# nipponjo/tts-arabic-pytorch

Hardware: AMD Instinct MI355X
Metric: audio samples/sec (FastPitch+HiFi-GAN, synthetic 64-phoneme inputs) (higher is better)
Workload: dtype f32

## Files before the change

include/ttsamd.h:

```cpp
#ifndef TTSAMD_H
#define TTSAMD_H

#include <stdint.h>

#ifdef __cplusplus
extern "C" {
#endif

#define TTSAMD_OK 0
#define TTSAMD_EINVAL (-1)
#define TTSAMD_EHIP (-2)
#define TTSAMD_ENOMEM (-3)

typedef struct ttsamd_tensor {
    const char* name;
    const float* data;
    int32_t ndim;
    int64_t shape[4];
} ttsamd_tensor;

typedef struct ttsamd_hifigan_cfg {
    int32_t num_mels;
    int32_t upsample_initial_channel;
    int32_t n_ups;
// ... 273 lines not shown
int32_t ttsamd_conv_last_launch(int32_t* route, int32_t* ksplit);
int32_t ttsamd_conv1d_route(int32_t batch, int32_t cin, int32_t cout, int32_t k, int32_t dilation, int32_t lin, float in_slope,
                            int32_t relu_out, int32_t has_res, int32_t mode, int64_t splitk_floats, int32_t* route, int32_t* ksplit);
int64_t ttsamd_convt_packed_floats(int32_t cin, int32_t cout, int32_t u);
int64_t ttsamd_convt_wino_packed_floats(int32_t cin, int32_t cout, int32_t u);
int32_t ttsamd_convt_wino_pack_weight(const float* w, const float* bias, int32_t cin, int32_t cout, int32_t u, float* out);
int32_t ttsamd_conv_transpose1d(const float* x, const float* w, const float* bias, const int64_t* lens, int32_t batch, int32_t cin,
                                int32_t cout, int32_t u, int32_t lin, float in_slope, float* y, float* packed, void* stream);

int64_t ttsamd_resblock_pair_packed_floats(int32_t channels, int32_t k, int32_t variant);
int32_t ttsamd_resblock_pair(const float* x, float* y, const float* w1, const float* b1, const float* w2, const float* b2,
                             int32_t channels, int32_t k, int32_t dil, const int64_t* lens, int32_t len_mul, int32_t L,
                             int32_t batch, int32_t mode, float div, float slope, int32_t variant, float* packed, int64_t packed_floats,
                             void* stream);

int64_t ttsamd_resblock2_packed_floats(int32_t channels, int32_t k, int32_t variant);
int32_t ttsamd_resblock2(const float* x, float* y, const float* w1, const float* b1, const float* w2, const float* b2, int32_t channels,
                         int32_t k, int32_t dil1, int32_t dil2, const int64_t* lens, int32_t len_mul, int32_t L, int32_t batch, int32_t mode,
                         float div, float slope, int32_t variant, float* packed, int64_t packed_floats, void* stream);

int32_t ttsamd_bfo_pack(const float* x, int32_t batch, int32_t channels, int32_t len, float slope, void* out, void* stream);
int32_t ttsamd_bfo_unpack(const void* in, int32_t batch, int32_t channels, int32_t len, float slope, float* out, void* stream);
int64_t ttsamd_bfo_weight_elems(int32_t cout, int32_t cin, int32_t k, int32_t up);
int32_t ttsamd_bfo_pack_weight(const float* w, int32_t cout, int32_t cin, int32_t k, int32_t up, uint16_t* out);
int32_t ttsamd_bfo_conv1d(const void* x, const void* w_packed, const float* bias, const void* res, const void* sum_in,
                          const int64_t* lens, int32_t len_mul, int32_t batch, int32_t cin, int32_t cout, int32_t k,
                          int32_t dilation, int32_t up, int32_t len_in, int32_t mode, float div, float res_slope,
                          float out_slope, void* y, float* y_f32, const float* res_f32, void* stream);
int32_t ttsamd_bfo_resblock_pair(const void* x, const void* w1, const float* b1, const void* w2, const float* b2,
                                 const void* sum_in, const int64_t* lens, int32_t len_mul, int32_t batch, int32_t channels,
// ... 125 lines not shown
```

tts-arabic-pytorch_amd/csrc/api.hip:

```cpp
#include <cerrno>
#include <cstdio>
#include <cstdlib>
#include <cstring>
#include <algorithm>
#include <atomic>
#include <mutex>
#include <string>
#include <vector>

#include "kernels.hpp"

namespace ttsamd {

static thread_local std::string g_err;

void set_error(const char* fmt, ...) {
    char buf[1024];
    va_list ap;
    va_start(ap, fmt);
    vsnprintf(buf, sizeof(buf), fmt, ap);
    va_end(ap);
    g_err = buf;
}

// ... 1009 lines not shown
                               channels, k, channels, packed + 2 * n + i * nw44);
            TTS_CHECK_HIP(hipGetLastError());
        }
        rc = launch_fused_pair4(channels, x, y, packed + 2 * n, b1, packed + 2 * n + nw44, b2, k, dil, lens, len_mul, L, batch, mode, div,
                                slope, s, 7);
    } else if (variant == -1) {
        rc = 0;
    } else {
        set_error("resblock_pair: variant %d (1: first generation, 2 / 3: second generation with 256- / 128-column blocks, 4 / 5: 256 columns + Winograd phase B / both phases, 6: C = 32 with both phases on Winograd F(4,3), 7: ... on its seven-point groups, k = 7 / 11)", variant);
        rc = TTSAMD_EINVAL;
    }
    prof_end(s);
    return rc;
}

int64_t ttsamd_resblock2_packed_floats(int32_t channels, int32_t k, int32_t variant) {
    if (channels < 1 || k < 1 || (variant != 1 && variant != 2)) return 0;
    return 2 * (int64_t)channels * k * channels;
}

int32_t ttsamd_resblock2(const float* x, float* y, const float* w1, const float* b1, const float* w2, const float* b2, int32_t channels,
                         int32_t k, int32_t dil1, int32_t dil2, const int64_t* lens, int32_t len_mul, int32_t L, int32_t batch, int32_t mode,
                         float div, float slope, int32_t variant, float* packed, int64_t packed_floats, void* stream) {
    TTS_REQUIRE(x && y && w1 && b1 && w2 && b2 && packed && channels % 32 == 0 && channels >= 32 && k >= 1 && batch >= 1 && L >= 1 &&
                len_mul >= 1 && mode >= 0 && mode <= 2 && x != y, "resblock2: bad argument");
    TTS_REQUIRE(variant == 1 || variant == 2, "resblock2: variant %d (1: two single-conv launches, 2: both convs in one launch)", variant);
    TTS_REQUIRE(packed_floats >= ttsamd_resblock2_packed_floats(channels, k, variant),
                "resblock2: `packed` holds %lld floats, C = %d, k = %d needs %lld (ttsamd_resblock2_packed_floats)", (long long)packed_floats,
                channels, k, (long long)ttsamd_resblock2_packed_floats(channels, k, variant));
    if (variant == 1) {
// ... 82 lines not shown
```

tts-arabic-pytorch_amd/csrc/common.hpp:

```cpp
#pragma once
#include <hip/hip_runtime.h>
#include <stdint.h>
#include <atomic>
#include <cstdarg>
#include <cstdio>
#include <cstdlib>
#include <string>

#include "../../include/ttsamd.h"

namespace ttsamd {

void set_error(const char* fmt, ...);

#define TTS_CHECK_HIP(expr)                                                         \
    do {                                                                            \
        hipError_t e_ = (expr);                                                     \
        if (e_ != hipSuccess) {                                                     \
            ttsamd::set_error("%s failed: %s (%s:%d)", #expr, hipGetErrorString(e_), \
                              __FILE__, __LINE__);                                  \
            return TTSAMD_EHIP;                                                     \
        }                                                                           \
    } while (0)

// ... 21 lines not shown
    e = hipFuncSetAttribute(fn, hipFuncAttributeMaxDynamicSharedMemorySize, bytes);
    if (e == hipSuccess && dev >= 0 && dev < 64) done.fetch_or(1ull << dev, std::memory_order_release);
    return e;
}

#define TTS_OPTIONS(X)                                                                                     \
    X(HIFIGAN_STREAMS, 0, 0, 1)    \
    X(WINO, 0, 0, 1)                                              \
    X(WINO2, 0, 0, 31)             \
    X(WINO4, 0, 0, 255)            \
    X(FUSED_PAIR, 0, 0, 1)                   \
    X(FUSED2, 0, 0, 1)                                           \
    X(FUSED2_MASK, 1, 0, 0x1ff)               \
    X(FUSED2_MASK_N1, 1, 0, 0x1ff)          \
    X(FUSED2_WB, 0, 0, 2)                     \
    X(PAIR4, 0, 0, 2)              \
    X(CONVT, 0, 0, 1)                              \
    X(CONVT_WINO, 0, 0, 2)         \
    X(BFO, 0, 0, 1)                \
    X(BFO_CHAIN, 0, 0, 1)                           \
    X(BFO_CHAIN7, 0, 0, 1)                                 \
    X(BFO_FF, 0, 0, 1)                              \
    X(BFO_SPLITK, 0, 0, 1)                                              \
    X(BFO_SMALL_TILES, 0, 0, 1)            \
    X(BF16_ATTN, 0, 0, 1)                                         \
    X(BF16_PACKED_T, 0, 0, 1)                   \
    X(ATT_RA, 0, 1, 4)                             \
    X(ATT_SPLIT, 0, 0, 1)                      \
    X(XCD_W, 0, 0, 1)                            \
    X(XCD_WMAX_KB, 0, 0, 1 << 20)     \
    X(DEEP_SPLITK, 0, 0, 1)        \
// ... 98 lines not shown
                         int u, int kt, int L, int len_mul, float in_slope, bool convt_ok, hipStream_t stream, const float* w_wino = nullptr,
                         const float* bias_wino = nullptr);
bool convt_wino_packable(int cin, int cout, int u);
void pack_convt_wino_weight(const float* w, const float* bias, int cin, int cout, int u, float* out_w, float* out_bias);
bool convt_wino_supported(const ConvParams& p, const float* w_wino, const float* bias_wino);
int32_t launch_convt_wino(const ConvParams& p, const float* w_wino, const float* bias_wino, hipStream_t stream);
bool fused_pair_supported(int32_t channels, int32_t k, int32_t dil, int32_t L, const float* x, const float* y);
int32_t launch_fused_pair(int32_t channels, const float* x, float* y, const float* w1, const float* b1, const float* w2,
                          const float* b2, int32_t k, int32_t dil, const int64_t* lens, int32_t len_mul, int32_t L, int32_t batch,
                          int32_t mode, float div, float slope, hipStream_t stream);
bool fused_pair2_supported(int32_t channels, int32_t k, int32_t dil, int32_t L, const float* x, const float* y, int32_t ntw);
int32_t launch_fused_pair2(int32_t channels, const float* x, float* y, const float* w1, const float* b1, const float* w2,
                           const float* b2, int32_t k, int32_t dil, const int64_t* lens, int32_t len_mul, int32_t L, int32_t batch,
                           int32_t mode, float div, float slope, int32_t ntw, hipStream_t stream, const float* w2_wino = nullptr,
                           const float* w1_wino = nullptr);
bool fused_pair4_supported(int32_t channels, int32_t k, int32_t dil, int32_t L, const float* x, const float* y);
int32_t launch_fused_pair4(int32_t channels, const float* x, float* y, const float* w1_wino4, const float* b1, const float* w2_wino4,
                           const float* b2, int32_t k, int32_t dil, const int64_t* lens, int32_t len_mul, int32_t L, int32_t batch,
                           int32_t mode, float div, float slope, hipStream_t stream, int32_t points = 6);
bool resblock2_conv_supported(int32_t channels, int32_t k, int32_t dil, int32_t L, const float* x, const float* y);
int32_t launch_resblock2_conv(int32_t channels, const float* x, float* y, const float* w, const float* b, int32_t k, int32_t dil,
                              const int64_t* lens, int32_t len_mul, int32_t L, int32_t batch, int32_t mode, float div, float slope,
                              hipStream_t stream);
bool resblock2_pair_supported(int32_t channels, int32_t k, int32_t d1, int32_t d2, int32_t L, const float* x, const float* y);
int32_t launch_resblock2_pair(int32_t channels, const float* x, float* y, const float* w1, const float* b1, const float* w2,
                              const float* b2, int32_t k, int32_t d1, int32_t d2, const int64_t* lens, int32_t len_mul, int32_t L,
                              int32_t batch, int32_t mode, float div, float slope, hipStream_t stream);
int32_t launch_wino(const ConvParams& p, hipStream_t stream);
void pack_wino_weight(const float* w, int cout, int cin, float* out);
int wino2_groups(int k);
// ... 64 lines not shown
```

tts-arabic-pytorch_amd/csrc/hifigan.hip:

```cpp
#include <cmath>
#include <cstring>
#include <cstdlib>
#include <map>
#include <mutex>
#include <string>
#include <vector>

#include "kernels.hpp"
#include "bfo.hpp"

namespace ttsamd {

constexpr unsigned kFused2Mask = 0x00F;
constexpr int kPair4MinK = 7;
constexpr unsigned kPair44Mask = 0x3;
constexpr unsigned kFused2MaskN1 = 0x000;
constexpr int64_t kFused2SmallColumns = 2 * 256 * 252;

constexpr unsigned kResblock2PairMask = 0x00;

static bool resblock2_pair_choice(unsigned mask, int32_t channels, int32_t k, int32_t d1, int32_t d2, int32_t L, const float* x,
                                  const float* y) {
    const int ci = channels == 32 ? 0 : (channels == 64 ? 1 : -1);
    const int ki = k == 3 ? 0 : (k == 5 ? 1 : (k == 7 ? 2 : -1));
    if (ci < 0 || ki < 0 || !(mask & (1u << (3 * ci + ki)))) return false;
    return resblock2_pair_supported(channels, k, d1, d2, L, x, y);
}

struct ConvW {
    int64_t w_off = 0, b_off = 0;
// ... 392 lines not shown
    struct Join {
        bool on; hipStream_t a, b;
        ~Join() { if (on) { (void)hipStreamSynchronize(a); (void)hipStreamSynchronize(b); } }
    } join{false, bs[1], bs[2]};
    const auto fail = [&](int32_t rc) { join.on = multi && rc != 0; return rc; };

    ConvParams p;
    std::memset(&p, 0, sizeof(p));
    p.batch = B;
    p.lens_in = lens; p.lens_out = lens;
    p.n_phase = 1; p.div = 1.f;
    p.splitk_ws = splitks[0]; p.splitk_floats = kSplitKFloats;
    const bool pack_t = default_precision() == 1 && opt_int(OPT_BF16_PACKED_T, 1) != 0;
    const Fused2Switches f2sw = read_fused2_switches();
    const bool fused_ok = default_precision() == 0 && opt_int(OPT_FUSED_PAIR, 1) != 0;
    const bool convt_ok = opt_int(OPT_CONVT, 1) != 0;
    const unsigned rb2_mask = (unsigned)opt_int(OPT_RESBLOCK2_PAIR, kResblock2PairMask);
    bool in_section = false;
    int pack_io = 0;
    auto conv = [&](const ConvW& cw, const float* x, hipStream_t st, float* y, const float* res, int L, int mul,
                    int dil, float slope, int mode, float div) -> int32_t {
        p.x = x; p.x_bs = (int64_t)cw.cin * L; p.x_cs = L;
        p.w = h->dev + cw.w_off; p.bias = h->dev + cw.b_off;
        p.w_bf16 = h->dev16 + cw.w16_off; p.precision = default_precision();
        p.w_wino = cw.ww_off >= 0 ? h->dev + cw.ww_off : nullptr;
        p.w_wino4 = (cw.ww4_off >= 0 && cw.cout >= 64) ? h->dev + cw.ww4_off : nullptr;
        p.w_wino44 = (cw.ww44_off >= 0 && cw.cout >= 64) ? h->dev + cw.ww44_off : nullptr;
        p.y = y; p.y_bs = (int64_t)cw.cout * L; p.y_cs = L; p.y_ts = 1;
        p.res = res; p.r_bs = (int64_t)cw.cout * L; p.r_cs = L;
        p.len_in_mul = mul; p.len_out_mul = mul; p.Lin = L; p.Nout = L;
// ... 172 lines not shown
                if (multi && j > 0) HG_CHECK_HIP(hipStreamWaitEvent(st, h->ev_done[j - 1], 0));
                if (in_section) prof_add(fl); else prof_begin(st, fl);
                rc2 = launch_resblock2_conv(w2.cin, Tb, cur, h->dev + w2.w_off, h->dev + w2.b_off, w2.k, d2, lens, mul, L, B, mode, div,
                                            0.1f, st);
                if (!in_section) prof_end(st);
                HG_TRY(rc2);
            }
            if (multi) HG_CHECK_HIP(hipEventRecord(h->ev_done[j], st));
        }
        for (int j = 0; !h->rb2 && j < cfg.n_kernels; ++j) {
            hipStream_t st = bs[j % 3];
            float *Tb = Tbs[j % 3], *R = Rs[j % 3];
            p.splitk_ws = splitks[j % 3];
            if (multi && j > 0) HG_CHECK_HIP(hipStreamWaitEvent(st, h->ev_fork, 0));
            const float* src = ups_out;
            for (int m = 0; m < cfg.n_dilations; ++m) {
                const int li = (i * cfg.n_kernels + j) * cfg.n_dilations + m;
                const int d = cfg.resblock_dilations[j][m];
                {
                    const bool last = m + 1 == cfg.n_dilations;
                    float* dst = last ? cur : (src == R ? Tb : R);
                    const ConvW &w1 = h->c1[li], &w2 = h->c2[li];
                    const bool square = w1.cin == w1.cout && w2.cin == w1.cin && w2.cout == w1.cin && w1.k == w2.k;
                    const int ntw2 = (fused_ok && square) ? fused2_choice(f2sw, w1.cin, w1.k, d, L, src, dst, (int64_t)B * L) : 0;
                    const bool f43 = ntw2 == 2 && f2sw.pair4 && f2sw.wino_a && w1.k >= kPair4MinK && w1.ww4_off >= 0 && w2.ww4_off >= 0 &&
                                     fused_pair4_supported(w1.cin, w1.k, d, L, src, dst);
                    const bool f44 = f43 && f2sw.pair44 && (kPair44Mask & (w1.k == 7 ? 1u : (w1.k == 11 ? 2u : 0u))) != 0 &&
                                     w1.ww44_off >= 0 && w2.ww44_off >= 0;
                    if (ntw2 != 0 || (fused_ok && square && fused_pair_supported(w1.cin, w1.k, d, L, src, dst))) {
                        const int mode = !last ? 0 : (cfg.n_kernels == 1 ? 0 : (j == 0 ? 0 : (j + 1 < cfg.n_kernels ? 1 : 2)));
// ... 64 lines not shown
```

tts-arabic-pytorch_amd/csrc/resblock_fused2.hip:

```cpp
#include <algorithm>
#include <cstdlib>
#include <cstring>

#include "conv_mfma_common.hpp"

namespace ttsamd {

struct FusedPair2Params {
    const float* x;
    float* y;
    const float4* w1;
    const float4* w2;
    const float4* w1w;
    const float4* w2w;
    const float* b1;
    const float* b2;
    const int64_t* lens;
    int32_t len_mul, L, dil, batch;
    int32_t mode;
    float div, slope;
    int32_t compact;
};

template <int K, int C, int NTW>
// ... 64 lines not shown
                }
            }
#pragma unroll
            for (int pq = 0; pq < 4; ++pq)
#pragma unroll
                for (int mt = 0; mt < MT; ++mt) {
                    const float av = pq == 0 ? a4[mt].x : (pq == 1 ? a4[mt].y : (pq == 2 ? a4[mt].z : a4[mt].w));
#pragma unroll
                    for (int j = 0; j < NTW; ++j)
                        acc[mt][j] = __builtin_amdgcn_mfma_f32_32x32x2f32(av, bv[j][pq], acc[mt][j], 0, 0, 0);
                }
        }
    }
}

template <int K, int C, bool EO, int MTW>
__device__ __forceinline__ void conv_phase2_wino(f32x16 (&acc)[4][MTW], float4 (&aq)[2][MTW], const float4* sb,
                                                 const float4* __restrict__ wl, const int rstride, const int cstep,
                                                 const float4* __restrict__ wnext) {
    using G = Fused2Geo<K, C, 2>;
    constexpr int NOCT = G::NOCT, MT = MTW, PF = G::PF, NS = G::NS, NL = G::NL, NGW = G::NGW, TSH = G::TSH;
    constexpr int NBU = NS + NL;
    constexpr int NGT = NOCT * NGW;
    typedef float f32x4v __attribute__((ext_vector_type(4)));
#define TTS_ENT(SBO, CC) (SBO)[EO ? ((CC) & 1) * TSH + ((CC) >> 1) : (CC) * cstep]
    float4 bq[2][4];
#pragma unroll
    for (int m = 0; m < 4; ++m) bq[0][m] = TTS_ENT(sb, m);
#pragma unroll 1
    for (int o = 0; o < NOCT; ++o) {
        const float4* sbo = sb + o * 2 * rstride;
        const float4* sbn = sb + min(o + 1, NOCT - 1) * 2 * rstride;
#pragma unroll
        for (int u = 0; u < NBU; ++u) {
// ... 1 lines not shown
            {
                const int un = u + 1;
                if (un < NS) {
#pragma unroll
                    for (int m = 0; m < 4; ++m) bq[nxt][m] = TTS_ENT(sbo, 3 * un + m);
                } else if (un < NBU) {
                    bq[nxt][0] = TTS_ENT(sbo, 3 * NS + (un - NS));
                    bq[nxt][1] = TTS_ENT(sbo, 3 * NS + (un - NS) + 1);
                } else {
#pragma unroll
                    for (int m = 0; m < 4; ++m) bq[nxt][m] = TTS_ENT(sbn, m);
                }
            }
            f32x4v x[4], v[4];
#pragma unroll
            for (int m = 0; m < 4; ++m) x[m] = f32x4v{bq[cur][m].x, bq[cur][m].y, bq[cur][m].z, bq[cur][m].w};
            const bool sub = u < NS;
            if (sub) { v[0] = x[0] - x[2]; v[1] = x[1] + x[2]; v[2] = x[2] - x[1]; v[3] = x[1] - x[3]; }
            else { v[0] = x[0]; v[1] = x[1]; }
            const int ng = sub ? 4 : 2;
            const int g0 = sub ? 4 * u : 4 * NS + 2 * (u - NS);
#pragma unroll
            for (int i = 0; i < ng; ++i) {
                const int g = g0 + i;
                const int plane = sub ? i : (i ? 3 : 0);
                const int slot = g % PF;
                float4 a4[MT];
#pragma unroll
                for (int mt = 0; mt < MT; ++mt) a4[mt] = aq[slot][mt];
                {
                    const int gn = o * NGW + g + PF;
// ... 426 lines not shown
        if (k == 7) return launch_fused2_k<7, 128, 2, 2>(p, stream);
        if (k == 11) return launch_fused2_k<11, 128, 2, 2>(p, stream);
    }
#define TTS_F2(KK, CC, NN) if (k == KK && channels == CC && ntw == NN) return launch_fused2_k<KK, CC, NN, 0>(p, stream);
    TTS_F2(3, 32, 2) TTS_F2(7, 32, 2) TTS_F2(11, 32, 2)
    TTS_F2(3, 64, 2) TTS_F2(7, 64, 2) TTS_F2(11, 64, 2)
    TTS_F2(3, 128, 2) TTS_F2(7, 128, 2) TTS_F2(11, 128, 2)
    TTS_F2(3, 32, 1) TTS_F2(7, 32, 1) TTS_F2(11, 32, 1)
    TTS_F2(3, 64, 1) TTS_F2(7, 64, 1) TTS_F2(11, 64, 1)
    TTS_F2(3, 128, 1) TTS_F2(7, 128, 1) TTS_F2(11, 128, 1)
#undef TTS_F2
    set_error("fused ResBlock pair (direct weights): no instantiation for C=%d, k=%d, ntw=%d", channels, k, ntw);
    return TTSAMD_EINVAL;
}

}
```

tts-arabic-pytorch_amd/ttsamd/engine.py:

```python
import ctypes as C

import numpy as np
import torch

from . import lib as L
from .config import NET_CONFIG, HIFIGAN_CONFIG, VOCOS_22K_CONFIG, TACOTRON2_CONFIG


def _require_gpu():
    if not torch.cuda.is_available():
        raise L.TtsAmdError('no ROCm device visible: the ttsamd engines run only on an MI355X (gfx950); '
                            'there is no CPU fallback')
    lib = L.load()
    if not lib.ttsamd_device_ok():
        raise L.TtsAmdError('device 0 is not gfx950')
    return lib


PRECISIONS = {'f32': 0, 'bf16': 1, 'bf16x3': 2}


def set_precision(name):
    lib = L.load()
    L.check(lib.ttsamd_set_precision(PRECISIONS[name]), 'set_precision')
# ... 640 lines not shown
    assert tuple(w1.shape) == tuple(w2.shape) == (Cc, Cc, k)
    if y is None:
        assert mode == 0
        y = torch.zeros_like(x)
    if lens is not None:
        lens = lens.to(device=x.device, dtype=torch.int64).contiguous()
    n_packed = int(lib.ttsamd_resblock_pair_packed_floats(Cc, k, int(variant)))
    packed = torch.empty(max(n_packed, 1), dtype=torch.float32, device=x.device)
    with torch.cuda.device(x.device):
        L.check(lib.ttsamd_resblock_pair(_ptr(x), _ptr(y), _ptr(w1), _ptr(b1), _ptr(w2), _ptr(b2), Cc, k, int(dil), _ptr(lens),
                                         int(len_mul), Lx, B, int(mode), float(div), float(slope), int(variant), _ptr(packed),
                                         n_packed, _stream()), 'resblock_pair')
    return y


def resblock2(x, w1, b1, w2, b2, dil1, dil2, lens=None, len_mul=1, y=None, mode=0, div=1.0, slope=0.1, variant=2):
    lib = _require_gpu()
    x = x.contiguous().float()
    w1, w2, b1, b2 = (t.contiguous().float() for t in (w1, w2, b1, b2))
    B, Cc, Lx = x.shape
    k = w1.shape[2]
    assert tuple(w1.shape) == tuple(w2.shape) == (Cc, Cc, k)
    if y is None:
        assert mode == 0
        y = torch.zeros_like(x)
    if lens is not None:
        lens = lens.to(device=x.device, dtype=torch.int64).contiguous()
    n_packed = int(lib.ttsamd_resblock2_packed_floats(Cc, k, int(variant)))
    packed = torch.empty(max(n_packed, 1), dtype=torch.float32, device=x.device)
    with torch.cuda.device(x.device):
        L.check(lib.ttsamd_resblock2(_ptr(x), _ptr(y), _ptr(w1), _ptr(b1), _ptr(w2), _ptr(b2), Cc, k, int(dil1), int(dil2), _ptr(lens),
# ... 1115 lines not shown
```

tts-arabic-pytorch_amd/ttsamd/lib.py:

```python
import ctypes as C
import os

_HERE = os.path.dirname(os.path.abspath(__file__))
LIB_PATH = os.environ.get('TTSAMD_LIB') or os.path.join(_HERE, 'lib', 'libttsamd.so')


class TtsAmdError(RuntimeError):
    pass


class Tensor(C.Structure):
    _fields_ = [('name', C.c_char_p), ('data', C.POINTER(C.c_float)), ('ndim', C.c_int32),
                ('shape', C.c_int64 * 4)]


class HifiGanCfg(C.Structure):
    _fields_ = [('num_mels', C.c_int32), ('upsample_initial_channel', C.c_int32), ('n_ups', C.c_int32),
                ('upsample_rates', C.c_int32 * 8), ('upsample_kernel_sizes', C.c_int32 * 8),
                ('n_kernels', C.c_int32), ('resblock_kernel_sizes', C.c_int32 * 8),
                ('n_dilations', C.c_int32), ('resblock_dilations', (C.c_int32 * 8) * 8), ('resblock', C.c_int32)]


class FastPitchCfg(C.Structure):
    _fields_ = [(n, C.c_int32) for n in (
# ... 147 lines not shown
    'ttsamd_tagger_destroy': (_I32, [_P]),
    'ttsamd_tagger_workspace_bytes': (_I64, [_P, _I32, _I32]),
    'ttsamd_tagger_forward': (_I32, [_P, _P, _I32, _I32, _P, _P, _I64, _P]),
    'ttsamd_conv1d_packed_floats': (_I64, [_I32, _I32, _I32]),
    'ttsamd_conv1d': (_I32, [_P, _P, _P, _P, _I32, _I32, _I32, _I32, _I32, _I32, _F, _I32, _P, _P, _P]),
    'ttsamd_conv1d_ex': (_I32, [_P, _P, _P, _P, _P, _I32, _I32, _I32, _I32, _I32, _I32, _F, _I32, _I32, _F, _P, _P, _P]),
    'ttsamd_conv1d_splitk': (_I32, [_P, _P, _P, _P, _P, _I32, _I32, _I32, _I32, _I32, _I32, _F, _I32, _I32, _F, _P, _P, _P, _I64, _P]),
    'ttsamd_conv_last_launch': (_I32, [C.POINTER(_I32), C.POINTER(_I32)]),
    'ttsamd_conv1d_route': (_I32, [_I32, _I32, _I32, _I32, _I32, _I32, _F, _I32, _I32, _I32, _I64, C.POINTER(_I32), C.POINTER(_I32)]),
    'ttsamd_convt_packed_floats': (_I64, [_I32, _I32, _I32]),
    'ttsamd_conv_transpose1d': (_I32, [_P, _P, _P, _P, _I32, _I32, _I32, _I32, _I32, _F, _P, _P, _P]),
    'ttsamd_convt_wino_packed_floats': (_I64, [_I32, _I32, _I32]),
    'ttsamd_convt_wino_pack_weight': (_I32, [_P, _P, _I32, _I32, _I32, _P]),
    'ttsamd_resblock_pair_packed_floats': (_I64, [_I32, _I32, _I32]),
    'ttsamd_resblock_pair': (_I32, [_P, _P, _P, _P, _P, _P, _I32, _I32, _I32, _P, _I32, _I32, _I32, _I32, _F, _F, _I32, _P, _I64, _P]),
    'ttsamd_resblock2_packed_floats': (_I64, [_I32, _I32, _I32]),
    'ttsamd_resblock2': (_I32, [_P, _P, _P, _P, _P, _P, _I32, _I32, _I32, _I32, _P, _I32, _I32, _I32, _I32, _F, _F, _I32, _P, _I64, _P]),
    'ttsamd_set_precision': (_I32, [_I32]),
    'ttsamd_get_precision': (_I32, []),
    'ttsamd_dp_unique_id': (_I32, [_P]),
    'ttsamd_dp_init': (_I32, [_I32, _I32, _P, C.POINTER(_P)]),
    'ttsamd_dp_destroy': (_I32, [_P]),
    'ttsamd_dp_rank': (_I32, [_P]),
    'ttsamd_dp_world': (_I32, [_P]),
    'ttsamd_dp_broadcast': (_I32, [_P, _P, _I64, _I32, _P]),
    'ttsamd_dp_broadcast_weights': (_I32, [_P, _I32, _P, _I32, _P]),
    'ttsamd_dp_allgather': (_I32, [_P, _P, _P, _I64, _P]),
    'ttsamd_dp_pack_audio': (_I32, [_P, _I64, _P, _I32, _I64, _P, _P]),
    'ttsamd_dp_gather_audio': (_I32, [_P, _P, _P, C.POINTER(_I64), C.POINTER(_I64), _I32, _P]),
    'ttsamd_profile_enable': (_I32, [_I32]),
# ... 109 lines not shown
```

Before: 79.67 million.

## Fuse three ResBlock dilation pairs into one chained kernel with halo tiles

Adds a kernel that runs all three conv pairs of a k=3 HiFi-GAN ResBlock (C=32/64) in one launch. Each block keeps a 256-column window with a 12-column halo in LDS, so intermediate activations never go back to global memory between pairs. The default mask enables it for both channel counts in the HiFi-GAN forward. The cost is halo recomputation (about 10% redundant columns) and higher register and LDS pressure, which may cut occupancy.

```diff
diff --git a/include/ttsamd.h b/include/ttsamd.h
--- a/include/ttsamd.h
+++ b/include/ttsamd.h
@@ -311,6 +311,13 @@
                              int32_t batch, int32_t mode, float div, float slope, int32_t variant, float* packed, int64_t packed_floats,
                              void* stream);
 
+int64_t ttsamd_resblock_chain_packed_floats(int32_t channels, int32_t k);
+int32_t ttsamd_resblock_chain_tile(int32_t* block, int32_t* halo, int32_t* stored);
+int32_t ttsamd_resblock_chain(const float* x, float* y, const float* const* w1, const float* const* b1, const float* const* w2,
+                              const float* const* b2, int32_t channels, int32_t k, const int32_t* dilations, const int64_t* lens,
+                              int32_t len_mul, int32_t L, int32_t batch, int32_t mode, float div, float slope, float* packed,
+                              int64_t packed_floats, void* stream);
+
 int64_t ttsamd_resblock2_packed_floats(int32_t channels, int32_t k, int32_t variant);
 int32_t ttsamd_resblock2(const float* x, float* y, const float* w1, const float* b1, const float* w2, const float* b2, int32_t channels,
                          int32_t k, int32_t dil1, int32_t dil2, const int64_t* lens, int32_t len_mul, int32_t L, int32_t batch, int32_t mode,
diff --git a/profiles/r36/chain_classes.py b/profiles/r36/chain_classes.py
--- /dev/null
+++ b/profiles/r36/chain_classes.py
@@ -0,0 +1,64 @@
+import csv
+import glob
+import os
+import re
+import sys
+from collections import defaultdict
+
+PAT = [(re.compile(r'resblock_pair2<3, (32|64), 2, 2>'), 'pair2<3,{},2,2>'), (re.compile(r'resblock_chain2<(32|64)>'), 'chain2<{}>')]
+
+
+def cls(name):
+    for pat, fmt in PAT:
+        m = pat.search(name)
+        if m:
+            return fmt.format(m.group(1))
+    return 'conv1d_wino4_f32 (control)' if 'conv1d_wino4_f32' in name else None
+
+
+def files(src, tail):
+    return [src] if src.endswith('.csv') else sorted(glob.glob(os.path.join(src, '**', '*' + tail), recursive=True))
+
+
+def trace(src, steps):
+    d = defaultdict(lambda: [0, 0])
+    for f in files(src, 'kernel_trace.csv'):
+        for r in csv.DictReader(open(f)):
+            c = cls(r['Kernel_Name'])
+            if c:
+                d[c][0] += 1
+                d[c][1] += int(r['End_Timestamp']) - int(r['Start_Timestamp'])
+    print(f'# {os.path.basename(os.path.normpath(src))} ({steps} calls of the step)')
+    for c in sorted(d):
+        n, t = d[c]
+        print(f'{c:28s} launches {n:5d}  us per launch {t / n / 1e3:8.1f}  ms per step {t / steps / 1e6:8.3f}')
+
+
+def pmc(src):
+    acc = defaultdict(lambda: defaultdict(float))
+    ids = defaultdict(set)
+    for f in files(src, 'counter_collection.csv'):
+        for r in csv.DictReader(open(f)):
+            c = cls(r['Kernel_Name'])
+            if c and 'control' not in c:
+                acc[c][r['Counter_Name']] += float(r['Counter_Value'])
+                ids[c].add(r['Dispatch_Id'])
+    print(f'# {os.path.basename(os.path.normpath(src))}')
+    for c in sorted(acc):
+        n = len(ids[c])
+        line = f'{c:18s} launches {n:3d} '
+        for k, v in sorted(acc[c].items()):
+            line += f' {k} per launch {v / n / 1024:9.1f} MB' if k.endswith('_SIZE') else f' {k} {v / n:.4g}'
+        v = acc[c]
+        if v.get('SQ_BUSY_CU_CYCLES') and 'SQ_VALU_MFMA_BUSY_CYCLES' in v:
+            line += f"  MfmaUtil {100 * v['SQ_VALU_MFMA_BUSY_CYCLES'] / (4 * v['SQ_BUSY_CU_CYCLES']):.1f} %"
+        print(line)
+
+
+if __name__ == '__main__':
+    if sys.argv[1] == 'trace':
+        for s in sys.argv[2:]:
+            trace(s, 9)
+    else:
+        for s in sys.argv[2:]:
+            pmc(s)
diff --git a/tts-arabic-pytorch_amd/csrc/api.hip b/tts-arabic-pytorch_amd/csrc/api.hip
--- a/tts-arabic-pytorch_amd/csrc/api.hip
+++ b/tts-arabic-pytorch_amd/csrc/api.hip
@@ -1047,6 +1047,49 @@
     return rc;
 }
 
+int64_t ttsamd_resblock_chain_packed_floats(int32_t channels, int32_t k) {
+    if (channels < 1 || !(k == 3 || k == 7 || k == 11)) return 0;
+    return 6 * (int64_t)channels * wino2_groups(k) * channels;
+}
+
+int32_t ttsamd_resblock_chain_tile(int32_t* block, int32_t* halo, int32_t* stored) {
+    TTS_REQUIRE(block && halo && stored, "resblock_chain_tile: null argument");
+    *block = kChain2Block; *halo = kChain2Halo; *stored = kChain2Stored;
+    return 0;
+}
+
+int32_t ttsamd_resblock_chain(const float* x, float* y, const float* const* w1, const float* const* b1, const float* const* w2,
+                              const float* const* b2, int32_t channels, int32_t k, const int32_t* dilations, const int64_t* lens,
+                              int32_t len_mul, int32_t L, int32_t batch, int32_t mode, float div, float slope, float* packed,
+                              int64_t packed_floats, void* stream) {
+    TTS_REQUIRE(x && y && w1 && b1 && w2 && b2 && dilations && packed && batch >= 1 && L >= 1 && len_mul >= 1 && mode >= 0 && mode <= 2,
+                "resblock_chain: bad argument");
+    TTS_REQUIRE(fused_chain2_supported(channels, k, dilations, 3, L, x, y),
+                "resblock_chain: C = %d, k = %d, dilations %d / %d / %d, L = %d is not covered (C = 32 / 64, k = 3, dilations out of 1 / 3 / 5 "
+                "with sum (d + 1) <= %d, L a multiple of 4, x != y, both 16-byte aligned)", channels, k, dilations[0], dilations[1],
+                dilations[2], L, kChain2Halo);
+    TTS_REQUIRE(packed_floats >= ttsamd_resblock_chain_packed_floats(channels, k),
+                "resblock_chain: `packed` holds %lld floats, C = %d, k = %d needs %lld (ttsamd_resblock_chain_packed_floats)",
+                (long long)packed_floats, channels, k, (long long)ttsamd_resblock_chain_packed_floats(channels, k));
+    hipStream_t s = (hipStream_t)stream;
+    const int64_t nw = (int64_t)channels * wino2_groups(k) * channels;
+    const float *w1w[3], *w2w[3];
+    for (int m = 0; m < 3; ++m) {
+        TTS_REQUIRE(w1[m] && w2[m] && b1[m] && b2[m], "resblock_chain: null filter or bias of pair %d", m);
+        for (int i = 0; i < 2; ++i) {
+            float* wino = packed + (2 * m + i) * nw;
+            hipLaunchKernelGGL(pack_wino2_weight_kernel, dim3((unsigned)((nw + 255) / 256)), dim3(256), 0, s, i == 0 ? w1[m] : w2[m], channels,
+                               channels, k, channels, wino);
+            TTS_CHECK_HIP(hipGetLastError());
+            (i == 0 ? w1w : w2w)[m] = wino;
+        }
+    }
+    prof_begin(s, 3 * 2.0 * (2.0 * channels * channels * k));
+    const int32_t rc = launch_fused_chain2(channels, x, y, w1w, b1, w2w, b2, k, dilations, 3, lens, len_mul, L, batch, mode, div, slope, s);
+    prof_end(s);
+    return rc;
+}
+
 int64_t ttsamd_resblock2_packed_floats(int32_t channels, int32_t k, int32_t variant) {
     if (channels < 1 || k < 1 || (variant != 1 && variant != 2)) return 0;
     return 2 * (int64_t)channels * k * channels;
diff --git a/tts-arabic-pytorch_amd/csrc/common.hpp b/tts-arabic-pytorch_amd/csrc/common.hpp
--- a/tts-arabic-pytorch_amd/csrc/common.hpp
+++ b/tts-arabic-pytorch_amd/csrc/common.hpp
@@ -59,7 +59,8 @@
     X(FUSED2_MASK, 1, 0, 0x1ff)               \
     X(FUSED2_MASK_N1, 1, 0, 0x1ff)          \
     X(FUSED2_WB, 0, 0, 2)                     \
-    X(PAIR4, 0, 0, 2)              \
+    X(FUSED_CHAIN, 0, 0, 3)        \
+    X(PAIR4, 0, 0, 2)             \
     X(CONVT, 0, 0, 1)                              \
     X(CONVT_WINO, 0, 0, 2)         \
     X(BFO, 0, 0, 1)                \
@@ -188,6 +189,15 @@
                            const float* b2, int32_t k, int32_t dil, const int64_t* lens, int32_t len_mul, int32_t L, int32_t batch,
                            int32_t mode, float div, float slope, int32_t ntw, hipStream_t stream, const float* w2_wino = nullptr,
                            const float* w1_wino = nullptr);
+constexpr int kChain2Block = 256, kChain2Halo = 12, kChain2Stored = kChain2Block - 2 * kChain2Halo;
+constexpr int chain2_tiles(int n) { return (n + kChain2Stored - 1) / kChain2Stored; }
+constexpr int chain2_first_stored(int tile) { return tile * kChain2Stored; }
+constexpr int chain2_window_start(int tile) { return chain2_first_stored(tile) - kChain2Halo; }
+bool fused_chain2_supported(int32_t channels, int32_t k, const int32_t* dil, int32_t n_pairs, int32_t L, const float* x, const float* y);
+int32_t launch_fused_chain2(int32_t channels, const float* x, float* y, const float* const* w1_wino, const float* const* b1,
+                            const float* const* w2_wino, const float* const* b2, int32_t k, const int32_t* dil, int32_t n_pairs,
+                            const int64_t* lens, int32_t len_mul, int32_t L, int32_t batch, int32_t mode, float div, float slope,
+                            hipStream_t stream);
 bool fused_pair4_supported(int32_t channels, int32_t k, int32_t dil, int32_t L, const float* x, const float* y);
 int32_t launch_fused_pair4(int32_t channels, const float* x, float* y, const float* w1_wino4, const float* b1, const float* w2_wino4,
                            const float* b2, int32_t k, int32_t dil, const int64_t* lens, int32_t len_mul, int32_t L, int32_t batch,
diff --git a/tts-arabic-pytorch_amd/csrc/hifigan.hip b/tts-arabic-pytorch_amd/csrc/hifigan.hip
--- a/tts-arabic-pytorch_amd/csrc/hifigan.hip
+++ b/tts-arabic-pytorch_amd/csrc/hifigan.hip
@@ -14,6 +14,7 @@
 constexpr unsigned kFused2Mask = 0x00F;
 constexpr int kPair4MinK = 7;
 constexpr unsigned kPair44Mask = 0x3;
+constexpr unsigned kFusedChainMask = 0x3;
 constexpr unsigned kFused2MaskN1 = 0x000;
 constexpr int64_t kFused2SmallColumns = 2 * 256 * 252;
 
@@ -436,6 +437,7 @@
     const bool pack_t = default_precision() == 1 && opt_int(OPT_BF16_PACKED_T, 1) != 0;
     const Fused2Switches f2sw = read_fused2_switches();
     const bool fused_ok = default_precision() == 0 && opt_int(OPT_FUSED_PAIR, 1) != 0;
+    const unsigned chain_mask = (unsigned)opt_int(OPT_FUSED_CHAIN, kFusedChainMask);
     const bool convt_ok = opt_int(OPT_CONVT, 1) != 0;
     const unsigned rb2_mask = (unsigned)opt_int(OPT_RESBLOCK2_PAIR, kResblock2PairMask);
     bool in_section = false;
@@ -638,6 +640,35 @@
             p.splitk_ws = splitks[j % 3];
             if (multi && j > 0) HG_CHECK_HIP(hipStreamWaitEvent(st, h->ev_fork, 0));
             const float* src = ups_out;
+            {
+                const int li0 = (i * cfg.n_kernels + j) * cfg.n_dilations;
+                const ConvW& w0 = h->c1[li0];
+                const unsigned cbit = w0.cin == 32 ? 1u : (w0.cin == 64 ? 2u : 0u);
+                bool chained = fused_ok && (chain_mask & cbit) != 0 && cfg.n_dilations == 3 && w0.k == 3 && w0.k < kPair4MinK &&
+                               f2sw.wino_a && f2sw.wino_b;
+                int32_t dl[3] = {0, 0, 0};
+                const float *cw1[3], *cw2[3], *cb1[3], *cb2[3];
+                for (int m = 0; chained && m < 3; ++m) {
+                    const ConvW &w1 = h->c1[li0 + m], &w2 = h->c2[li0 + m];
+                    dl[m] = cfg.resblock_dilations[j][m];
+                    chained = w1.cin == w0.cin && w1.cout == w0.cin && w2.cin == w0.cin && w2.cout == w0.cin && w1.k == 3 && w2.k == 3 &&
+                              w1.ww_off >= 0 && w2.ww_off >= 0 && (dl[m] == 1 || dl[m] == 3 || dl[m] == 5) &&
+                              fused2_choice(f2sw, w0.cin, 3, dl[m], L, ups_out, cur, (int64_t)B * L) == 2;
+                    cw1[m] = h->dev + w1.ww_off; cw2[m] = h->dev + w2.ww_off; cb1[m] = h->dev + w1.b_off; cb2[m] = h->dev + w2.b_off;
+                }
+                if (chained && fused_chain2_supported(w0.cin, 3, dl, 3, L, ups_out, cur)) {
+                    const int mode = cfg.n_kernels == 1 ? 0 : (j == 0 ? 0 : (j + 1 < cfg.n_kernels ? 1 : 2));
+                    if (multi && j > 0 && mode != 0) HG_CHECK_HIP(hipStreamWaitEvent(st, h->ev_done[j - 1], 0));
+                    const double fl = 3 * 2.0 * (2.0 * w0.cin * w0.cin * 3) * mul;
+                    if (in_section) prof_add(fl); else prof_begin(st, fl);
+                    const int32_t crc = launch_fused_chain2(w0.cin, ups_out, cur, cw1, cb1, cw2, cb2, 3, dl, 3, lens, mul, L, B, mode,
+                                                            (float)cfg.n_kernels, 0.1f, st);
+                    if (!in_section) prof_end(st);
+                    HG_TRY(crc);
+                    if (multi) HG_CHECK_HIP(hipEventRecord(h->ev_done[j], st));
+                    continue;
+                }
+            }
             for (int m = 0; m < cfg.n_dilations; ++m) {
                 const int li = (i * cfg.n_kernels + j) * cfg.n_dilations + m;
                 const int d = cfg.resblock_dilations[j][m];
diff --git a/tts-arabic-pytorch_amd/csrc/resblock_fused2.hip b/tts-arabic-pytorch_amd/csrc/resblock_fused2.hip
--- a/tts-arabic-pytorch_amd/csrc/resblock_fused2.hip
+++ b/tts-arabic-pytorch_amd/csrc/resblock_fused2.hip
@@ -102,10 +102,10 @@
     }
 }
 
-template <int K, int C, bool EO, int MTW>
+template <int K, int C, bool EO, int MTW, bool ACT = false>
 __device__ __forceinline__ void conv_phase2_wino(f32x16 (&acc)[4][MTW], float4 (&aq)[2][MTW], const float4* sb,
                                                  const float4* __restrict__ wl, const int rstride, const int cstep,
-                                                 const float4* __restrict__ wnext) {
+                                                 const float4* __restrict__ wnext, const float slope = 1.f) {
     using G = Fused2Geo<K, C, 2>;
     constexpr int NOCT = G::NOCT, MT = MTW, PF = G::PF, NS = G::NS, NL = G::NL, NGW = G::NGW, TSH = G::TSH;
     constexpr int NBU = NS + NL;
@@ -137,7 +137,10 @@
             }
             f32x4v x[4], v[4];
 #pragma unroll
-            for (int m = 0; m < 4; ++m) x[m] = f32x4v{bq[cur][m].x, bq[cur][m].y, bq[cur][m].z, bq[cur][m].w};
+            for (int m = 0; m < 4; ++m) {
+                x[m] = f32x4v{bq[cur][m].x, bq[cur][m].y, bq[cur][m].z, bq[cur][m].w};
+                if (ACT) x[m] = f32x4v{lrelu_max(x[m][0], slope), lrelu_max(x[m][1], slope), lrelu_max(x[m][2], slope), lrelu_max(x[m][3], slope)};
+            }
             const bool sub = u < NS;
             if (sub) { v[0] = x[0] - x[2]; v[1] = x[1] + x[2]; v[2] = x[2] - x[1]; v[3] = x[1] - x[3]; }
             else { v[0] = x[0]; v[1] = x[1]; }
@@ -594,4 +597,303 @@
     return TTSAMD_EINVAL;
 }
 
-}
+struct FusedChain2Params {
+    const float* x;
+    float* y;
+    const float4* w1w[3];
+    const float4* w2w[3];
+    const float* b1[3];
+    const float* b2[3];
+    const int64_t* lens;
+    int32_t len_mul, L, batch;
+    int32_t dil[3];
+    int32_t mode;
+    float div, slope;
+    int32_t compact;
+};
+
+template <int C>
+struct Chain2Geo {
+    static constexpr int NB = kChain2Block, HALO = kChain2Halo, TS = kChain2Stored;
+    static constexpr int WS = 270;
+    static constexpr int WAVES = C == 32 ? 3 : 2;
+    static constexpr bool RAW = C == 64;
+    static size_t lds_bytes() { return (size_t)2 * (C / 8) * WS * sizeof(float4); }
+    static_assert(C * NB * 4 <= 2 * (C / 8) * WS * 16, "the epilogue's row buffer lies in the window");
+};
+
+template <int C>
+__global__ __launch_bounds__(256, Chain2Geo<C>::WAVES)
+void resblock_chain2(const FusedChain2Params p) {
+    using G = Fused2Geo<3, C, 2>;
+    using T = Chain2Geo<C>;
+    constexpr int NOCT = G::NOCT, MT = G::MT, PF = G::PF, TSH = G::TSH;
+    constexpr int NB = T::NB, HALO = T::HALO, TS = T::TS, WS = T::WS;
+    constexpr bool RAW = T::RAW;
+    extern __shared__ __attribute__((aligned(16))) float4 smem4[];
+    const int tid = threadIdx.x, lane = tid & 63, wid = tid >> 6;
+    const int kk = lane >> 5, l31 = lane & 31;
+    int b = blockIdx.z;
+    int tile = blockIdx.x;
+    if (p.compact) {
+        int t = 0;
+        if (!live_tile(p.lens, p.len_mul, p.L, TS, p.batch, blockIdx.z * gridDim.x + blockIdx.x, b, t)) return;
+        b = __builtin_amdgcn_readfirstlane(b);
+        tile = __builtin_amdgcn_readfirstlane(t);
+    }
+    int len = p.L;
+    if (p.lens) len = min(len, (int)p.lens[b] * p.len_mul);
+    if (chain2_first_stored(tile) >= len) return;
+    const int L = p.L;
+    const int P0 = chain2_window_start(tile);
+    const float slope = p.slope;
+    const float* __restrict__ xb = p.x + (int64_t)b * C * L;
+    float4* Xs = smem4;
+
+    const int wofs = kk * C + l31;
+    float4 aq[PF][MT];
+#pragma unroll
+    for (int g = 0; g < PF; ++g)
+#pragma unroll
+        for (int mt = 0; mt < MT; ++mt) aq[g][mt] = p.w1w[0][wofs + g * 2 * C + 32 * mt];
+
+    constexpr int n_ent = 2 * NOCT * WS;
+    {
+        constexpr int NE = (n_ent + 255) / 256;
+        float v[NE][4];
+        int eo[NE];
+        bool ok[NE];
+        int okk = 0, col = tid;
+        while (col >= WS) { col -= WS; ++okk; }
+#pragma unroll
+        for (int u = 0; u < NE; ++u) {
+            const int pos = P0 + col;
+            const int okc = min(okk, 2 * NOCT - 1);
+            ok[u] = col < NB && pos >= 0 && pos < len;
+            eo[u] = tid + 256 * u < n_ent ? okc * WS + col : -1;
+            const float* src = xb + (int64_t)((okc >> 1) * 8 + (okc & 1)) * L + min(max(pos, 0), len - 1);
+#pragma unroll
+            for (int pc = 0; pc < 4; ++pc) v[u][pc] = src[(int64_t)2 * pc * L];
+            col += 256;
+            while (col >= WS) { col -= WS; ++okk; }
+        }
+#pragma unroll
+        for (int u = 0; u < NE; ++u)
+            if (eo[u] >= 0) Xs[eo[u]] = ok[u] ? make_float4(v[u][0], v[u][1], v[u][2], v[u][3]) : make_float4(0.f, 0.f, 0.f, 0.f);
+    }
+    __syncthreads();
+
+    const int jw = wid * 32 + l31;
+    f32x16 res0[MT], res1[MT];
+    const auto residual_from_window = [&]() {
+#pragma unroll
+        for (int mt = 0; mt < MT; ++mt)
+#pragma unroll
+            for (int oc = 0; oc < 4; ++oc)
+#pragma unroll
+                for (int k2 = 0; k2 < 2; ++k2) {
+                    const float* src = reinterpret_cast<const float*>(Xs + ((4 * mt + oc) * 2 + k2) * WS + 2 * jw) + 2 * kk;
+                    const float2 r0 = *reinterpret_cast<const float2*>(src);
+                    const float2 r1 = *reinterpret_cast<const float2*>(src + 4);
+                    res0[mt][4 * oc + k2] = r0.x; res0[mt][4 * oc + k2 + 2] = r0.y;
+                    res1[mt][4 * oc + k2] = r1.x; res1[mt][4 * oc + k2 + 2] = r1.y;
+                }
+    };
+    if constexpr (!RAW) {
+        residual_from_window();
+        __syncthreads();
+        for (int e = tid; e < n_ent; e += 256) {
+            float4 v4 = Xs[e];
+            v4.x = lrelu_max(v4.x, slope); v4.y = lrelu_max(v4.y, slope); v4.z = lrelu_max(v4.z, slope); v4.w = lrelu_max(v4.w, slope);
+            Xs[e] = v4;
+        }
+        __syncthreads();
+    }
+
+    float* ep = reinterpret_cast<float*>(smem4);
+    const int pos0 = P0 + 2 * jw;
+    int lo = 0;
+#pragma unroll
+    for (int m = 0; m < 3; ++m) {
+        const int dil = p.dil[m];
+        const float4* __restrict__ wl1 = p.w1w[m] + wofs;
+        const float4* __restrict__ wl2 = p.w2w[m] + wofs;
+        const int npa = G::npa(dil);
+        const int pa = min(jw, npa - 1);
+        const int na = dil == 1 ? 2 * pa : (pa / dil) * 2 * dil + pa % dil;
+        {
+            f32x16 accA[4][MT];
+#pragma unroll
+            for (int mt = 0; mt < MT; ++mt)
+#pragma unroll
+                for (int r = 0; r < 16; ++r) {
+                    const float bv = p.b1[m][32 * mt + (r & 3) + 8 * (r >> 2) + 4 * kk];
+                    accA[0][mt][r] = bv; accA[1][mt][r] = 0.f; accA[2][mt][r] = 0.f; accA[3][mt][r] = -bv;
+                }
+            conv_phase2_wino<3, C, false, MT, RAW>(accA, aq, Xs + kk * WS + lo + na, wl1, WS, dil, wl2, slope);
+            if constexpr (RAW) residual_from_window();
+            __syncthreads();
+            if (jw < npa) {
+#pragma unroll
+                for (int hh = 0; hh < 2; ++hh) {
+                    const int u = lo + dil + na + hh * dil;
+                    const int c = u + 1;
+                    const int pos = P0 + u;
+                    const bool live = pos >= 0 && pos < len;
+                    const int ent = (c & 1) * TSH + (c >> 1);
+                    if (c < 2 * TSH) {
+#pragma unroll
+                        for (int mt = 0; mt < MT; ++mt)
+#pragma unroll
+                            for (int oc = 0; oc < 4; ++oc)
+#pragma unroll
+                                for (int k2 = 0; k2 < 2; ++k2) {
+                                    const int r = 4 * oc + k2;
+                                    float v0 = hh ? accA[1][mt][r] - accA[2][mt][r] - accA[3][mt][r] : accA[0][mt][r] + accA[1][mt][r] + accA[2][mt][r];
+                                    float v1 = hh ? accA[1][mt][r + 2] - accA[2][mt][r + 2] - accA[3][mt][r + 2]
+                                                  : accA[0][mt][r + 2] + accA[1][mt][r + 2] + accA[2][mt][r + 2];
+                                    v0 = lrelu_max(v0, slope);
+                                    v1 = lrelu_max(v1, slope);
+                                    const float2 w2v = live ? make_float2(v0, v1) : make_float2(0.f, 0.f);
+                                    *reinterpret_cast<float2*>(reinterpret_cast<float*>(Xs + ((4 * mt + oc) * 2 + k2) * 2 * TSH + ent) + 2 * kk) = w2v;
+                                }
+                    }
+                }
+            }
+            __syncthreads();
+        }
+        f32x16 accw[4][MT];
+#pragma unroll
+        for (int mt = 0; mt < MT; ++mt)
+#pragma unroll
+            for (int r = 0; r < 16; ++r) {
+                const float bv = p.b2[m][32 * mt + (r & 3) + 8 * (r >> 2) + 4 * kk];
+                accw[0][mt][r] = res0[mt][r] + bv; accw[1][mt][r] = 0.f; accw[2][mt][r] = 0.f; accw[3][mt][r] = -(res1[mt][r] + bv);
+            }
+        if (m == 2 && p.mode != 0) {
+            const int n = 2 * jw;
+            const int voff = ((n >= HALO && n < HALO + TS && pos0 < len) ? pos0 : 0) * 4 + 4 * kk * L * 4;
+            const auto ys = __builtin_amdgcn_make_buffer_rsrc(p.y + (int64_t)b * C * L, 0, C * L * 4, 0x00020000);
+#pragma unroll
+            for (int mt = 0; mt < MT; ++mt)
+#pragma unroll
+                for (int r = 0; r < 16; ++r) {
+                    const int so = (32 * mt + (r & 3) + 8 * (r >> 2)) * L * 4;
+                    accw[0][mt][r] += __builtin_bit_cast(float, __builtin_amdgcn_raw_buffer_load_b32(ys, voff, so, 0));
+                    accw[3][mt][r] -= __builtin_bit_cast(float, __builtin_amdgcn_raw_buffer_load_b32(ys, voff + 4, so, 0));
+                }
+        }
+        conv_phase2_wino<3, C, true, MT>(accw, aq, Xs + kk * 2 * TSH + jw, wl2, 2 * TSH, 0, m < 2 ? p.w1w[m < 2 ? m + 1 : 2] + wofs : nullptr);
+        __syncthreads();
+        if (m < 2) {
+            const bool live0 = pos0 >= 0 && pos0 < len, live1 = pos0 + 1 >= 0 && pos0 + 1 < len;
+#pragma unroll
+            for (int mt = 0; mt < MT; ++mt) {
+#pragma unroll
+                for (int r = 0; r < 16; ++r) {
+                    res0[mt][r] = accw[0][mt][r] + accw[1][mt][r] + accw[2][mt][r];
+                    res1[mt][r] = accw[1][mt][r] - accw[2][mt][r] - accw[3][mt][r];
+                }
+                const float sl = RAW ? 1.f : slope;
+#pragma unroll
+                for (int oc = 0; oc < 4; ++oc)
+#pragma unroll
+                    for (int k2 = 0; k2 < 2; ++k2) {
+                        const int r = 4 * oc + k2;
+                        float* dst = reinterpret_cast<float*>(Xs + ((4 * mt + oc) * 2 + k2) * WS + 2 * jw) + 2 * kk;
+                        *reinterpret_cast<float2*>(dst) = live0 ? make_float2(lrelu_max(res0[mt][r], sl), lrelu_max(res0[mt][r + 2], sl))
+                                                                : make_float2(0.f, 0.f);
+                        *reinterpret_cast<float2*>(dst + 4) = live1 ? make_float2(lrelu_max(res1[mt][r], sl), lrelu_max(res1[mt][r + 2], sl))
+                                                                    : make_float2(0.f, 0.f);
+                    }
+            }
+            __syncthreads();
+            lo += dil + 1;
+        } else {
+#pragma unroll
+            for (int mt = 0; mt < MT; ++mt)
+#pragma unroll
+                for (int r = 0; r < 16; ++r) {
+                    float2 y2;
+                    y2.x = accw[0][mt][r] + accw[1][mt][r] + accw[2][mt][r];
+                    y2.y = accw[1][mt][r] - accw[2][mt][r] - accw[3][mt][r];
+                    *reinterpret_cast<float2*>(ep + (32 * mt + (r & 3) + 8 * (r >> 2) + 4 * kk) * NB + 2 * jw) = y2;
+                }
+        }
+    }
+    __syncthreads();
+    const bool do_div = p.mode == 2;
+    const float div = p.div;
+    float* __restrict__ yb = p.y + (int64_t)b * C * L;
+    const int n = lane * 4;
+    const int q = P0 + n;
+    const int wid_u = __builtin_amdgcn_readfirstlane(wid);
+    if (n >= HALO && n < HALO + TS && q < len) {
+#pragma unroll 4
+        for (int it = 0; it < C / 4; ++it) {
+            const int ch = wid_u + 4 * it;
+            const float4 v4 = *reinterpret_cast<const float4*>(ep + ch * NB + n);
+            float vv[4] = {v4.x, v4.y, v4.z, v4.w};
+            if (do_div) {
+#pragma unroll
+                for (int e = 0; e < 4; ++e) vv[e] = vv[e] / div;
+            }
+            float* yp = yb + (int64_t)ch * L + q;
+            if (q + 3 < len) {
+                *reinterpret_cast<float4*>(yp) = make_float4(vv[0], vv[1], vv[2], vv[3]);
+            } else {
+#pragma unroll
+                for (int e = 0; e < 4; ++e)
+                    if (q + e < len) yp[e] = vv[e];
+            }
+        }
+    }
+}
+
+bool fused_chain2_supported(int32_t channels, int32_t k, const int32_t* dil, int32_t n_pairs, int32_t L, const float* x, const float* y) {
+    if (!(channels == 32 || channels == 64) || k != 3 || n_pairs != 3 || !dil) return false;
+    int halo = 0;
+    for (int m = 0; m < 3; ++m) {
+        if (!(dil[m] == 1 || dil[m] == 3 || dil[m] == 5)) return false;
+        halo += dil[m] + 1;
+    }
+    if (halo > kChain2Halo) return false;
+    if (L < 1 || (L & 3) != 0 || ((((uintptr_t)x) | ((uintptr_t)y)) & 15) != 0 || x == y) return false;
+    return (int64_t)channels * L * 4 < ((int64_t)1 << 31);
+}
+
+template <int C>
+static int32_t launch_chain2_c(const FusedChain2Params& p, hipStream_t stream) {
+    using T = Chain2Geo<C>;
+    static std::atomic<uint64_t> lds_done{0};
+    TTS_CHECK_HIP(lds_opt_in((const void*)resblock_chain2<C>, (int)T::lds_bytes(), lds_done));
+    dim3 grid((p.L + T::TS - 1) / T::TS, 1, p.batch);
+    hipLaunchKernelGGL((resblock_chain2<C>), grid, dim3(256), T::lds_bytes(), stream, p);
+    TTS_CHECK_HIP(hipGetLastError());
+    return 0;
+}
+
+int32_t launch_fused_chain2(int32_t channels, const float* x, float* y, const float* const* w1_wino, const float* const* b1,
+                            const float* const* w2_wino, const float* const* b2, int32_t k, const int32_t* dil, int32_t n_pairs,
+                            const int64_t* lens, int32_t len_mul, int32_t L, int32_t batch, int32_t mode, float div, float slope,
+                            hipStream_t stream) {
+    TTS_REQUIRE(fused_chain2_supported(channels, k, dil, n_pairs, L, x, y),
+                "chained ResBlock: unsupported geometry (C=%d, k=%d, %d pairs, L=%d; C = 32 / 64, k = 3, three dilations of 1 / 3 / 5 "
+                "with sum (d + 1) <= %d, L a multiple of 4, x != y, 16-byte aligned)", channels, k, n_pairs, L, kChain2Halo);
+    TTS_REQUIRE(slope > 0.f && slope <= 1.f, "chained ResBlock: leaky-relu slope %g outside (0, 1]", (double)slope);
+    TTS_REQUIRE(mode >= 0 && mode <= 2 && batch >= 1 && len_mul >= 1, "chained ResBlock: mode %d, batch %d, len_mul %d", mode, batch, len_mul);
+    conv_log("fused_chain2", k, channels, channels, L, batch, 1, mode, len_mul, lens != nullptr, 1);
+    FusedChain2Params p;
+    std::memset(&p, 0, sizeof(p));
+    p.x = x; p.y = y;
+    for (int m = 0; m < 3; ++m) {
+        TTS_REQUIRE(w1_wino[m] && w2_wino[m] && b1[m] && b2[m], "chained ResBlock: null filter or bias of pair %d", m);
+        p.w1w[m] = reinterpret_cast<const float4*>(w1_wino[m]); p.w2w[m] = reinterpret_cast<const float4*>(w2_wino[m]);
+        p.b1[m] = b1[m]; p.b2[m] = b2[m]; p.dil[m] = dil[m];
+    }
+    p.lens = lens; p.len_mul = len_mul; p.L = L; p.batch = batch; p.mode = mode; p.div = div; p.slope = slope;
+    p.compact = compact_order(lens, batch) ? 1 : 0;
+    return channels == 32 ? launch_chain2_c<32>(p, stream) : launch_chain2_c<64>(p, stream);
+}
+
+}
diff --git a/tts-arabic-pytorch_amd/ttsamd/engine.py b/tts-arabic-pytorch_amd/ttsamd/engine.py
--- a/tts-arabic-pytorch_amd/ttsamd/engine.py
+++ b/tts-arabic-pytorch_amd/ttsamd/engine.py
@@ -678,7 +678,36 @@
     return y
 
 
-def resblock2(x, w1, b1, w2, b2, dil1, dil2, lens=None, len_mul=1, y=None, mode=0, div=1.0, slope=0.1, variant=2):
+def resblock_chain_tile():
+    v = [C.c_int32(0) for _ in range(3)]
+    L.check(L.load().ttsamd_resblock_chain_tile(*[C.byref(t) for t in v]), 'resblock_chain_tile')
+    return tuple(int(t.value) for t in v)
+
+
+def resblock_chain(x, w1, b1, w2, b2, dilations, lens=None, len_mul=1, y=None, mode=0, div=1.0, slope=0.1):
+    lib = _require_gpu()
+    x = x.contiguous().float()
+    w1, b1, w2, b2 = ([t.contiguous().float() for t in ts] for ts in (w1, b1, w2, b2))
+    B, Cc, Lx = x.shape
+    k = w1[0].shape[2]
+    assert len(w1) == len(b1) == len(w2) == len(b2) == len(dilations) == 3
+    assert all(tuple(t.shape) == (Cc, Cc, k) for t in w1 + w2)
+    if y is None:
+        assert mode == 0
+        y = torch.zeros_like(x)
+    if lens is not None:
+        lens = lens.to(device=x.device, dtype=torch.int64).contiguous()
+    n_packed = int(lib.ttsamd_resblock_chain_packed_floats(Cc, k))
+    packed = torch.empty(max(n_packed, 1), dtype=torch.float32, device=x.device)
+    arr = lambda ts: (C.c_void_p * 3)(*[t.data_ptr() for t in ts])
+    dl = (C.c_int32 * 3)(*[int(d) for d in dilations])
+    with torch.cuda.device(x.device):
+        L.check(lib.ttsamd_resblock_chain(_ptr(x), _ptr(y), arr(w1), arr(b1), arr(w2), arr(b2), Cc, k, dl, _ptr(lens), int(len_mul), Lx,
+                                          B, int(mode), float(div), float(slope), _ptr(packed), n_packed, _stream()), 'resblock_chain')
+    return y
+
+
+def resblock2(x, w1, b1, w2, b2, dil1, dil2,lens=None, len_mul=1, y=None, mode=0, div=1.0, slope=0.1, variant=2):
     lib = _require_gpu()
     x = x.contiguous().float()
     w1, w2, b1, b2 = (t.contiguous().float() for t in (w1, w2, b1, b2))
diff --git a/tts-arabic-pytorch_amd/ttsamd/lib.py b/tts-arabic-pytorch_amd/ttsamd/lib.py
--- a/tts-arabic-pytorch_amd/ttsamd/lib.py
+++ b/tts-arabic-pytorch_amd/ttsamd/lib.py
@@ -185,6 +185,9 @@
     'ttsamd_convt_wino_pack_weight': (_I32, [_P, _P, _I32, _I32, _I32, _P]),
     'ttsamd_resblock_pair_packed_floats': (_I64, [_I32, _I32, _I32]),
     'ttsamd_resblock_pair': (_I32, [_P, _P, _P, _P, _P, _P, _I32, _I32, _I32, _P, _I32, _I32, _I32, _I32, _F, _F, _I32, _P, _I64, _P]),
+    'ttsamd_resblock_chain_packed_floats': (_I64, [_I32, _I32]),
+    'ttsamd_resblock_chain_tile': (_I32, [C.POINTER(_I32), C.POINTER(_I32), C.POINTER(_I32)]),
+    'ttsamd_resblock_chain': (_I32, [_P, _P, _P, _P, _P, _P, _I32, _I32, _P, _P, _I32, _I32, _I32, _I32, _F, _F, _P, _I64, _P]),
     'ttsamd_resblock2_packed_floats': (_I64, [_I32, _I32, _I32]),
     'ttsamd_resblock2': (_I32, [_P, _P, _P, _P, _P, _P, _I32, _I32, _I32, _I32, _P, _I32, _I32, _I32, _I32, _F, _F, _I32, _P, _I64, _P]),
     'ttsamd_set_precision': (_I32, [_I32]),
```

Result: no change. 80.29 million, median of 6 (+0.8%).
